# tyfeld/MMaDA-Parallel

Measured on NVIDIA B200. Metric: denoised_tokens_per_sec, higher is better.
Workload: dtype bf16

## Files before the change

### mmada_parallel_b200/csrc/gemm.cu

```cuda
#include "gemm_epilogue.cuh"

#include <stdlib.h>

#include <map>
#include <mutex>
#include <utility>

namespace mmdp {

static constexpr int BM = 128, BK = 64;
static constexpr int kABytes = BM * BK * 2;
static constexpr int kGemmThreads = 256;
template <int BN> struct GemmCfg {
    static constexpr int kBBytes = BN * BK * 2;
    static constexpr int kStageBytes = kABytes + kBBytes;
    static constexpr int kStages = (BN == 256) ? 4 : 5;
    static constexpr int kScatBytes = 4 * kScatStageFloats * 4;
    static constexpr int kSmem = kStages * kStageBytes + 1024  + 256  + kScatBytes;
};

template <int EPI, int BN>
__global__ void __launch_bounds__(kGemmThreads, 1)
gemm_bf16_kernel(const __grid_constant__ CUtensorMap tmA, const __grid_constant__ CUtensorMap tmB, const GemmParams p) {
    constexpr int kStages = GemmCfg<BN>::kStages;
// ... 192 lines not shown
void set_gemm_splitk_mode(int m) { set_opt("gemm_splitk", m); }

static GemmPlan plan_gemm(int epi, int M, int N, int K) {
    const int mode = gemm_splitk_mode();
    const int g = num_sms();
    const int num_k = (K + BK - 1) / BK;
    const bool flexible = epi == EPI_PLAIN || epi == EPI_RESID || epi == EPI_F32;
    const bool may_split = num_k >= 4 && (mode >= 2 || (mode == 1 && epi == EPI_RESID));
    GemmPlan best{256, 0, 0, 0, 0};
    double best_cost = 1e30;
    for (int bn : {256, 192}) {
        if (bn == 192 && !flexible) continue;
        const int tiles = ((M + BM - 1) / BM) * ((N + bn - 1) / bn);
        GemmPlan pl{bn, tiles < g ? tiles : g, 0, 0, 0};
        double waves;
        const int full = tiles >= g ? (tiles / g) * g : 0;
        const int tail = tiles - full;
        waves = (double)((tiles + g - 1) / g);
        if (may_split && tail > 0 && tail * 2 <= g) {
            int splits = g / tail;
            if (splits > num_k / 2) splits = num_k / 2;
            if (splits > kSkMaxSplits) splits = kSkMaxSplits;
            if (splits >= 2) {
                const int kb_per = (num_k + splits - 1) / splits;
                splits = (num_k + kb_per - 1) / kb_per;
                const double exch = mode >= 3 ? 0.0 : 12.0 / num_k + 0.04;
                const double split_waves = (double)(full / g) + (double)kb_per / num_k + exch;
                if (split_waves < waves) {
                    pl.tail = tail; pl.splits = splits; pl.kb_per = kb_per;
                    pl.grid = full > 0 ? g : tail * splits;
                    waves = split_waves;
                }
            }
        }
        const double cost = waves * bn * (bn == 192 ? 1.04 : 1.0);
        if (cost < best_cost) { best_cost = cost; best = pl; }
    }
    return best;
}

struct SkWorkspace { float* ws; int* cnt; };
static std::map<std::pair<int, cudaStream_t>, SkWorkspace> g_sk;
static std::mutex g_sk_mu;
static int splitk_workspace(cudaStream_t stream, SkWorkspace* out) {
    int dev = 0;
    MMDP_CUDA(cudaGetDevice(&dev));
    std::lock_guard<std::mutex> lk(g_sk_mu);
    auto key = std::make_pair(dev, stream);
    auto it = g_sk.find(key);
    if (it != g_sk.end()) { *out = it->second; return 0; }
    const size_t units = 256;
    SkWorkspace w{nullptr, nullptr};
    MMDP_CUDA(cudaMalloc(&w.ws, units * BM * 256 * sizeof(float)));
    MMDP_CUDA(cudaMalloc(&w.cnt, 2 * units * sizeof(int)));
    MMDP_CUDA(cudaMemsetAsync(w.cnt, 0, 2 * units * sizeof(int), stream));
    g_sk.emplace(key, w);
    *out = w;
    return 0;
}

int gemm_pair_mode() { return opt(OPT_GEMM_PAIR); }
void set_gemm_pair_mode(int on) { set_opt("gemm_pair", (on == 2) ? 2 : (on ? 1 : 0)); }

int gemm_bf16(int epi, const __nv_bfloat16* A, int lda, const __nv_bfloat16* W, int ldw, int M, int N, int K,
              __nv_bfloat16* C, int ldc, const __nv_bfloat16* resid, int ldr, const QkvRopeArgs* qa,
              cudaStream_t stream, const GemmScatter* sc) {
    if (sc && epi != EPI_F32) return set_error("gemm: the scatter epilogue belongs to MMDP_EPI_F32");
    if (sc && (sc->rows_per_rank <= 0 || sc->slot < 0 || sc->slot > 7 || (M + sc->rows_per_rank - 1) / sc->rows_per_rank > 8))
        return set_error("gemm: bad scatter layout");
    if (M <= 0 || N <= 0 || K <= 0) return set_error("gemm: empty problem");
    if ((lda % 8) || (ldw % 8) || (K % 8)) return set_error("gemm: lda/ldw/K must be multiples of 8 (16-byte TMA strides)");
    if ((reinterpret_cast<uintptr_t>(A) & 15) || (reinterpret_cast<uintptr_t>(W) & 15))
        return set_error("gemm: A/W must be 16-byte aligned");
    switch (epi) {
        case EPI_PLAIN:
            if (!C || (ldc % 8) || (N % 8)) return set_error("gemm: C null or ldc/N not multiple of 8");
            break;
        case EPI_RESID:
            if (!C || !resid || (ldc % 8) || (ldr % 8) || (N % 8)) return set_error("gemm: bad residual epilogue args");
            break;
        case EPI_F32:
            if ((!C && !sc) || (ldc % 4) || (N % 4)) return set_error("gemm: fp32 output needs ldc/N multiples of 4");
            break;
        case EPI_SWIGLU:
            if (!C || (ldc % 8) || (N % 256)) return set_error("gemm: swiglu needs N % 256 == 0 (interleaved gate/up tiles)");
            break;
        case EPI_QKVROPE:
            if (!qa) return set_error("gemm: qkv epilogue needs QkvRopeArgs");
            if (qa->d_model % 256 || N != 3 * qa->d_model || qa->d_model != qa->n_heads * 128)
                return set_error("gemm: qkv epilogue needs head_dim 128, d_model % 256 == 0, N == 3*d_model");
            if (qa->pos_map ? (qa->Tq <= 0 || M % qa->Tq) : (!qa->chunked && (M % qa->L))) return set_error("gemm: qkv epilogue needs M == B*L (or B*Tq with a position map)");
            break;
        default:
            return set_error("gemm: unknown epilogue");
    }
    const int pm = gemm_pair_mode();
    if ((pm == 1 && M > 256) || (pm == 2 && M >= 4096 && N >= 8192)) return gemm_bf16_pair(epi, A, lda, W, ldw, M, N, K, C, ldc, resid, ldr, qa, stream, sc);
    GemmParams p{};
    p.M = M; p.N = N; p.K = K;
    p.C = C; p.ldc = ldc; p.resid = resid; p.ldr = ldr;
    GemmPlan pl = plan_gemm(epi, M, N, K);
    if (qa && qa->pos_map && pl.tail > 0) {
        pl.tail = 0; pl.splits = 0; pl.kb_per = 0;
        const int t = ((M + BM - 1) / BM) * ((N + pl.bn - 1) / pl.bn);
        pl.grid = t < num_sms() ? t : num_sms();
    }
    if (sc) {
        if (pl.tail > 0) { pl.tail = 0; pl.splits = 0; pl.kb_per = 0; const int t = ((M + BM - 1) / BM) * ((N + pl.bn - 1) / pl.bn); pl.grid = t < num_sms() ? t : num_sms(); }
        for (int r = 0; r < 8; ++r) p.scat_dst[r] = sc->dst[r];
        p.scat_R = sc->rows_per_rank; p.scat_slot = sc->slot;
// ... 45 lines not shown
```

### mmada_parallel_b200/csrc/gemm2.cu

```cuda
#include "gemm_epilogue.cuh"

namespace mmdp {

static constexpr int P_BM = 128, P_BK = 64;
static constexpr int kPABytes = P_BM * P_BK * 2;
static constexpr int kPairThreads = 256;
template <int BN> struct PairCfg {
    static constexpr int kBHalfBytes = (BN / 2) * P_BK * 2;
    static constexpr int kStageBytes = kPABytes + kBHalfBytes;
    static constexpr int kStages = (BN == 256) ? 6 : 7;
    static constexpr int kSmem = kStages * kStageBytes + 1024 + 256 + 4 * kScatStageFloats * 4;
    template <int EPI> static constexpr bool can_split() { return BN == 256 && (EPI == EPI_PLAIN || EPI == EPI_RESID || EPI == EPI_QKVROPE); }
};

__device__ __forceinline__ uint32_t cluster_ctarank() {
    uint32_t r;
    asm volatile("mov.u32 %0, %%cluster_ctarank;" : "=r"(r));
    return r;
}
__device__ __forceinline__ void cluster_sync_all() {
    asm volatile("barrier.cluster.arrive.release.aligned;\n\tbarrier.cluster.wait.acquire.aligned;" ::: "memory");
}
__device__ __forceinline__ uint32_t mapa_u32(uint32_t smem_addr, uint32_t rank) {
    uint32_t r;
    asm volatile("mapa.shared::cluster.u32 %0, %1, %2;" : "=r"(r) : "r"(smem_addr), "r"(rank));
    return r;
}
__device__ __forceinline__ void mbar_arrive_cluster(uint32_t cluster_addr) {
    asm volatile("mbarrier.arrive.shared::cluster.b64 _, [%0];" ::"r"(cluster_addr) : "memory");
}
template <uint32_t kCols>
__device__ __forceinline__ void tmem_alloc_pair(uint32_t* smem_dst) {
    asm volatile("tcgen05.alloc.cta_group::2.sync.aligned.shared::cta.b32 [%0], %1;" ::"r"(smem_u32(smem_dst)), "n"(kCols) : "memory");
    asm volatile("tcgen05.relinquish_alloc_permit.cta_group::2.sync.aligned;" ::: "memory");
}
template <uint32_t kCols>
__device__ __forceinline__ void tmem_dealloc_pair(uint32_t taddr) {
    asm volatile("tcgen05.dealloc.cta_group::2.sync.aligned.b32 %0, %1;" ::"r"(taddr), "n"(kCols) : "memory");
}
__device__ __forceinline__ void tma_load_2d_pair(void* smem_dst, const CUtensorMap* tm, uint32_t leader_bar_cluster_addr, int c0, int c1) {
    asm volatile(
        "cp.async.bulk.tensor.2d.cta_group::2.shared::cluster.global.mbarrier::complete_tx::bytes [%0], [%1, {%3, %4}], [%2];"
        ::"r"(smem_u32(smem_dst)), "l"(reinterpret_cast<uint64_t>(tm)), "r"(leader_bar_cluster_addr), "r"(c0), "r"(c1)
        : "memory");
}
__device__ __forceinline__ void umma_bf16_ss_pair(uint32_t d_tmem, uint64_t a_desc, uint64_t b_desc, uint32_t idesc, uint32_t acc) {
    asm volatile(
        "{\n\t.reg .pred p;\n\t"
        "setp.ne.b32 p, %4, 0;\n\t"
        "tcgen05.mma.cta_group::2.kind::f16 [%0], %1, %2, %3, p;\n\t}"
        ::"r"(d_tmem), "l"(a_desc), "l"(b_desc), "r"(idesc), "r"(acc)
        : "memory");
}
__device__ __forceinline__ void umma_commit_pair(uint64_t* bar) {
    const uint16_t mask = 3;
    asm volatile("tcgen05.commit.cta_group::2.mbarrier::arrive::one.shared::cluster.multicast::cluster.b64 [%0], %1;"
                 ::"r"(smem_u32(bar)), "h"(mask)
                 : "memory");
}

template <int EPI, int BN>
__global__ void __cluster_dims__(2, 1, 1) __launch_bounds__(kPairThreads, 1)
gemm_pair_kernel(const __grid_constant__ CUtensorMap tmA, const __grid_constant__ CUtensorMap tmB,
                 const __grid_constant__ CUtensorMap tmBh, const __grid_constant__ CUtensorMap tmAh, const GemmParams p) {
    constexpr int kStages = PairCfg<BN>::kStages;
    constexpr int kStageBytes = PairCfg<BN>::kStageBytes;
    static_assert(EPI == EPI_PLAIN || EPI == EPI_RESID || EPI == EPI_F32 || BN == 256, "fused QKV / SwiGLU epilogues need 256-wide tiles");
    extern __shared__ uint8_t smem_raw[];
    uint8_t* smem = reinterpret_cast<uint8_t*>((reinterpret_cast<uintptr_t>(smem_raw) + 1023) & ~uintptr_t(1023));
    uint64_t* full_bar = reinterpret_cast<uint64_t*>(smem + kStages * kStageBytes);
    uint64_t* empty_bar = full_bar + kStages;
    uint64_t* tmem_full = empty_bar + kStages;
    uint64_t* tmem_empty = tmem_full + 2;
    uint32_t* tmem_ptr = reinterpret_cast<uint32_t*>(tmem_empty + 2);
    float* scat_stage = reinterpret_cast<float*>(smem + kStages * kStageBytes + 256);

    const int warp = threadIdx.x >> 5;
    const int lane = threadIdx.x & 31;
    const uint32_t rank = cluster_ctarank();
    const bool leader = rank == 0;

    if (warp == 0 && lane == 0) {
        tma_prefetch_desc(&tmA);
        tma_prefetch_desc(&tmB);
    }
    if (warp == 1 && lane == 0) {
        for (int s = 0; s < kStages; ++s) {
            mbar_init(&full_bar[s], 2);
            mbar_init(&empty_bar[s], 1);
        }
        for (int s = 0; s < 2; ++s) {
            mbar_init(&tmem_full[s], 1);
            mbar_init(&tmem_empty[s], 8);
        }
        fence_barrier_init();
    }
    cluster_sync_all();
    if (warp == 2) tmem_alloc_pair<512>(tmem_ptr);
    tcgen05_fence_before();
    cluster_sync_all();
    tcgen05_fence_after();
    const uint32_t tmem_base = *tmem_ptr;
    pdl_launch_dependents();
    pdl_wait();

    const int num_m = (p.M + 2 * P_BM - 1) / (2 * P_BM);
    const int num_n = (p.N + BN - 1) / BN;
    const int num_k = (p.K + P_BK - 1) / P_BK;
    const int num_tiles = num_m * num_n;
    const int cluster_id = blockIdx.x >> 1, num_clusters = gridDim.x >> 1;
    constexpr bool kCanSplit = PairCfg<BN>::template can_split<EPI>();
    const int t_full = kCanSplit ? num_tiles - p.nsplit_tail : num_tiles;
    const int num_units = t_full + 2 * (num_tiles - t_full);
    constexpr bool kMTail = EPI == EPI_SWIGLU && BN == 256;
    auto decode = [&](int unit, int& m_blk, int& n_blk, bool& mhalf) {
        n_blk = unit / num_m;
        const int o = unit - n_blk * num_m;
        mhalf = false;
        m_blk = o;
        if (kMTail && p.mtail) {
            const int sp = (n_blk / p.mt_period) % num_m;
            mhalf = o == sp;
            m_blk = mhalf ? num_m - 1 : (o < sp ? o : o - 1);
        }
    };

    if (warp == 0) {
        if (elect_one_sync()) {
            int s = 0;
            uint32_t ph = 0;
            for (int unit = cluster_id; unit < num_units; unit += num_clusters) {
                const bool half = kCanSplit && unit >= t_full;
                const int tile = half ? t_full + ((unit - t_full) >> 1) : unit;
                int m_blk, n_blk;
                bool mhalf;
                decode(tile, m_blk, n_blk, mhalf);
                const int row0 = mhalf ? m_blk * 2 * P_BM + (int)rank * (P_BM / 2) : m_blk * 2 * P_BM + (int)rank * P_BM;
                const int wrow0 = half ? n_blk * BN + ((unit - t_full) & 1) * (BN / 2) + (int)rank * (BN / 4) : n_blk * BN + (int)rank * (BN / 2);
                const uint32_t tx = half ? 2 * (kPABytes + PairCfg<BN>::kBHalfBytes / 2)
                                         : (mhalf ? 2 * (kPABytes / 2 + PairCfg<BN>::kBHalfBytes) : 2 * kStageBytes);
                for (int kb = 0; kb < num_k; ++kb) {
                    mbar_wait(&empty_bar[s], ph ^ 1);
                    const uint32_t leader_full = mapa_u32(smem_u32(&full_bar[s]), 0);
                    if (leader) {
                        mbar_expect_tx(&full_bar[s], tx);
                    } else {
                        mbar_arrive_cluster(leader_full);
                    }
                    uint8_t* sa = smem + s * kStageBytes;
                    if (kMTail && mhalf) {
                        tma_load_2d_pair(sa, &tmAh, leader_full, kb * P_BK, row0);
                        tma_load_2d_pair(sa + kPABytes, &tmBh, leader_full, kb * P_BK, n_blk * BN + (int)rank * (BN / 4));
                        tma_load_2d_pair(sa + kPABytes + PairCfg<BN>::kBHalfBytes / 2, &tmBh, leader_full, kb * P_BK, n_blk * BN + BN / 2 + (int)rank * (BN / 4));
                    } else {
                        tma_load_2d_pair(sa, &tmA, leader_full, kb * P_BK, row0);
                        tma_load_2d_pair(sa + kPABytes, half ? &tmBh : &tmB, leader_full, kb * P_BK, wrow0);
                    }
                    if (++s == kStages) { s = 0; ph ^= 1; }
                }
            }
        }
        __syncwarp();
    } else if (warp == 1) {
        if (leader && elect_one_sync()) {
            constexpr uint32_t idesc_whole = umma_idesc_bf16(2 * P_BM, BN);
            constexpr uint32_t idesc_half = umma_idesc_bf16(2 * P_BM, kCanSplit ? BN / 2 : BN);
            int s = 0;
            uint32_t ph = 0;
            int as = 0;
            uint32_t aph = 0;
            constexpr uint32_t idesc_mhalf = umma_idesc_bf16(P_BM, BN);
            for (int unit = cluster_id; unit < num_units; unit += num_clusters) {
                uint32_t idesc = (kCanSplit && unit >= t_full) ? idesc_half : idesc_whole;
                if (kMTail && p.mtail) {
                    int m_blk, n_blk;
                    bool mhalf;
                    decode(unit, m_blk, n_blk, mhalf);
                    if (mhalf) idesc = idesc_mhalf;
                }
                mbar_wait(&tmem_empty[as], aph ^ 1);
                tcgen05_fence_after();
                const uint32_t d_tmem = tmem_base + as * BN;
                for (int kb = 0; kb < num_k; ++kb) {
                    mbar_wait(&full_bar[s], ph);
                    tcgen05_fence_after();
                    const uint32_t sa = smem_u32(smem + s * kStageBytes);
                    const uint64_t adesc = umma_desc_kmajor_sw128(sa);
                    const uint64_t bdesc = umma_desc_kmajor_sw128(sa + kPABytes);
#pragma unroll
                    for (int k = 0; k < P_BK / 16; ++k)
                        umma_bf16_ss_pair(d_tmem, adesc + (k * 2), bdesc + (k * 2), idesc, (kb | k) != 0);
                    umma_commit_pair(&empty_bar[s]);
                    if (kb == num_k - 1) umma_commit_pair(&tmem_full[as]);
                    if (++s == kStages) { s = 0; ph ^= 1; }
                }
                if (++as == 2) { as = 0; aph ^= 1; }
            }
        }
        __syncwarp();
    } else if (warp >= 4) {
        const int ew = warp - 4;
        int as = 0;
        uint32_t aph = 0;
        for (int unit = cluster_id; unit < num_units; unit += num_clusters) {
            const bool half = kCanSplit && unit >= t_full;
            const int tile = half ? t_full + ((unit - t_full) >> 1) : unit;
            int m_blk, n_blk;
            bool mhalf;
            decode(tile, m_blk, n_blk, mhalf);
            mbar_wait(&tmem_full[as], aph);
            tcgen05_fence_after();
            const uint32_t tbase = tmem_base + (static_cast<uint32_t>(ew * 32) << 16) + as * BN;
            if (kMTail && mhalf) {
                const int ln = ew * 32 + lane, hq = ln >> 6;
                const int row = m_blk * 2 * P_BM + (int)rank * (P_BM / 2) + (ln & 63);
                const bool row_ok = row < p.M;
#pragma unroll 1
                for (int c = 0; c < 2; ++c) {
                    uint32_t g[32], u[32];
                    tmem_ld_32x32b_x32(tbase + c * 32, g);
                    tmem_ld_32x32b_x32(tbase + 64 + c * 32, u);
                    tmem_ld_wait();
                    swiglu_store32(p, g, u, row, row_ok, n_blk * 128 + hq * 64 + c * 32);
                }
            } else {
            const int row = m_blk * 2 * P_BM + (int)rank * P_BM + ew * 32 + lane;
            const bool row_ok = row < p.M;
            if constexpr (kCanSplit) {
                if (half)
                    gemm_epilogue_tile<EPI, BN / 2>(p, tbase, row, row_ok, 2 * n_blk + ((unit - t_full) & 1), scat_stage + ew * kScatStageFloats);
                else
                    gemm_epilogue_tile<EPI, BN>(p, tbase, row, row_ok, n_blk, scat_stage + ew * kScatStageFloats);
            } else {
                gemm_epilogue_tile<EPI, BN>(p, tbase, row, row_ok, n_blk, scat_stage + ew * kScatStageFloats);
            }
            }
            tcgen05_fence_before();
            __syncwarp();
            if (lane == 0) mbar_arrive_cluster(mapa_u32(smem_u32(&tmem_empty[as]), 0));
            if (++as == 2) { as = 0; aph ^= 1; }
        }
        if constexpr (EPI == EPI_F32) {
            if (p.scat_R > 0) __threadfence_system();
        }
    }

    tcgen05_fence_before();
    cluster_sync_all();
    if (warp == 2) {
        tcgen05_fence_after();
        tmem_dealloc_pair<512>(tmem_base);
    }
}

template <int EPI, int BN>
static int launch_pair(const CUtensorMap& tmA, const CUtensorMap& tmB, const CUtensorMap& tmBh, const CUtensorMap& tmAh, GemmParams& p, cudaStream_t stream) {
    static unsigned long long attr_set = 0;
    int dev = 0;
    MMDP_CUDA(cudaGetDevice(&dev));
    if (!(attr_set >> (dev & 63) & 1ull)) {
        MMDP_CUDA(cudaFuncSetAttribute(gemm_pair_kernel<EPI, BN>, cudaFuncAttributeMaxDynamicSharedMemorySize, PairCfg<BN>::kSmem));
        attr_set |= 1ull << (dev & 63);
    }
    const int num_tiles = ((p.M + 2 * P_BM - 1) / (2 * P_BM)) * ((p.N + BN - 1) / BN);
    const int pairs = num_sms() / 2;
    const int grid = 2 * (num_tiles < pairs ? num_tiles : pairs);
    const int tail = num_tiles % pairs;
    p.nsplit_tail = (PairCfg<BN>::template can_split<EPI>() && opt(OPT_GEMM_NSPLIT_TAIL) && num_tiles > pairs && tail > 0 &&
                     2 * tail <= pairs && p.N % BN == 0) ? tail : 0;
    const int num_m = (p.M + 2 * P_BM - 1) / (2 * P_BM), m_rem = p.M - (num_m - 1) * 2 * P_BM;
    p.mtail = (EPI == EPI_SWIGLU && BN == 256 && opt(OPT_GEMM_MTAIL) && num_m >= 2 && m_rem <= P_BM && p.N % BN == 0 && num_tiles > pairs) ? 1 : 0;
    if (p.mtail) {
        int a = num_m, b = pairs;
        while (b) { const int t = a % b; a = b; b = t; }
        p.mt_period = pairs / a;
    }
    LaunchScope ls(LK_GEMM, 2.0 * p.M * (double)p.N * p.K, stream);
    MMDP_CUDA(launch_ex(gemm_pair_kernel<EPI, BN>, dim3(grid), dim3(kPairThreads), PairCfg<BN>::kSmem, stream, pdl_mode() != 0, false, tmA, tmB,
                        (p.nsplit_tail || p.mtail) ? tmBh : tmB, p.mtail ? tmAh : tmA, p));
    return 0;
}

static int pick_pair_tile_n(int M, int N) {
    const int g = num_sms() / 2;
    const long long m_tiles = (M + 2 * P_BM - 1) / (2 * P_BM);
    const long long w256 = (m_tiles * ((N + 255) / 256) + g - 1) / g * 256 * 100;
    const long long w192 = (m_tiles * ((N + 191) / 192) + g - 1) / g * 192 * 102;
    return w192 < w256 ? 192 : 256;
}

int gemm_bf16_pair(int epi, const __nv_bfloat16* A, int lda, const __nv_bfloat16* W, int ldw, int M, int N, int K,
                   __nv_bfloat16* C, int ldc, const __nv_bfloat16* resid, int ldr, const QkvRopeArgs* qa, cudaStream_t stream,
                   const GemmScatter* sc) {
    GemmParams p{};
    p.M = M; p.N = N; p.K = K;
    p.C = C; p.ldc = ldc; p.resid = resid; p.ldr = ldr;
    if (sc) {
        for (int r = 0; r < 8; ++r) p.scat_dst[r] = sc->dst[r];
        p.scat_R = sc->rows_per_rank; p.scat_slot = sc->slot;
    }
    const int bn = (epi == EPI_PLAIN || epi == EPI_RESID || epi == EPI_F32) ? pick_pair_tile_n(M, N) : 256;
    CUtensorMap tmA, tmB;
    if (make_tmap_2d_bf16(&tmA, A, (uint64_t)M, (uint64_t)K, (uint64_t)lda, P_BM, P_BK)) return -1;
    if (make_tmap_2d_bf16(&tmB, W, (uint64_t)N, (uint64_t)K, (uint64_t)ldw, bn / 2, P_BK)) return -1;
    CUtensorMap tmBh = tmB;
    if (bn == 256 && epi != EPI_F32 && make_tmap_2d_bf16(&tmBh, W, (uint64_t)N, (uint64_t)K, (uint64_t)ldw, bn / 4, P_BK)) return -1;
    CUtensorMap tmAh = tmA;
    if (epi == EPI_SWIGLU && make_tmap_2d_bf16(&tmAh, A, (uint64_t)M, (uint64_t)K, (uint64_t)lda, P_BM / 2, P_BK)) return -1;
    switch (epi) {
        case EPI_PLAIN:
            return bn == 192 ? launch_pair<EPI_PLAIN, 192>(tmA, tmB, tmBh, tmAh, p, stream) : launch_pair<EPI_PLAIN, 256>(tmA, tmB, tmBh, tmAh, p, stream);
        case EPI_RESID:
            return bn == 192 ? launch_pair<EPI_RESID, 192>(tmA, tmB, tmBh, tmAh, p, stream) : launch_pair<EPI_RESID, 256>(tmA, tmB, tmBh, tmAh, p, stream);
        case EPI_F32:
            return bn == 192 ? launch_pair<EPI_F32, 192>(tmA, tmB, tmBh, tmAh, p, stream) : launch_pair<EPI_F32, 256>(tmA, tmB, tmBh, tmAh, p, stream);
        case EPI_SWIGLU:
            return launch_pair<EPI_SWIGLU, 256>(tmA, tmB, tmBh, tmAh, p, stream);
        case EPI_QKVROPE:
            p.q = qa->q; p.k = qa->k; p.vt = qa->vt; p.cos_tab = qa->cos_tab; p.sin_tab = qa->sin_tab;
            p.L = qa->L; p.Lpad = qa->Lpad; p.d_model = qa->d_model; p.n_heads = qa->n_heads;
            p.pos_map = qa->pos_map; p.Tq = qa->Tq; p.row0 = qa->row0;
            return launch_pair<EPI_QKVROPE, 256>(tmA, tmB, tmBh, tmAh, p, stream);
        default:
            return set_error("gemm_pair: unknown epilogue");
    }
}

}
```

### mmada_parallel_b200/csrc/gemm_epilogue.cuh

```cuda
#pragma once
#include "mmdp_internal.h"
#include "ptx.cuh"

namespace mmdp {

struct GemmParams {
    int M, N, K;
    __nv_bfloat16* C;
    int ldc;
    const __nv_bfloat16* resid;
    int ldr;
    __nv_bfloat16* q;
    __nv_bfloat16* k;
    __nv_bfloat16* vt;
    const float* cos_tab;
    const float* sin_tab;
    int L, Lpad, d_model, n_heads;
    const int* pos_map;
    int Tq;
    int row0;
    int sk_tail, sk_splits, sk_kb_per;
    float* sk_ws;
    int* sk_cnt;
    int l2pf, l2pf_mod;
    float* scat_dst[8];
    int scat_R, scat_slot;
    int group_m;
    int nsplit_tail;
    int mtail, mt_period;
};

__host__ __device__ __forceinline__ void gemm_tile_coords(int tl, int num_m, int num_n, int group_m, int& m_blk, int& n_blk) {
    if (group_m <= 0 || group_m >= num_m) {
        m_blk = tl % num_m;
        n_blk = tl / num_m;
    } else {
        const int per_group = group_m * num_n;
        const int gid = tl / per_group, r = tl - gid * per_group;
        const int first = gid * group_m;
        const int gsz = (num_m - first < group_m) ? num_m - first : group_m;
        m_blk = first + r % gsz;
        n_blk = r / gsz;
    }
}

__device__ __forceinline__ void store_bf16x32(__nv_bfloat16* dst, const uint32_t (&p)[16], int ncols_valid) {
    uint4* d4 = reinterpret_cast<uint4*>(dst);
#pragma unroll
    for (int i = 0; i < 4; ++i) {
        if (i * 8 < ncols_valid) d4[i] = make_uint4(p[4 * i], p[4 * i + 1], p[4 * i + 2], p[4 * i + 3]);
    }
}

__device__ __forceinline__ void swiglu_store32(const GemmParams& p, const uint32_t (&g)[32], const uint32_t (&u)[32], int row, bool row_ok, int col0) {
    const int nvalid = p.N / 2 - col0;
    if (row_ok && nvalid > 0) {
        uint32_t pk[16];
#pragma unroll
        for (int i = 0; i < 16; ++i) {
            float o[2];
#pragma unroll
            for (int h = 0; h < 2; ++h) {
                float gg = bf16_round(__uint_as_float(g[2 * i + h]));
                float uu = bf16_round(__uint_as_float(u[2 * i + h]));
                float s = bf16_round(__fdiv_rn(gg, __fadd_rn(1.0f, expf(-gg))));
                o[h] = __fmul_rn(s, uu);
            }
            pk[i] = pack_bf16x2(o[0], o[1]);
        }
        store_bf16x32(p.C + (size_t)row * p.ldc + col0, pk, nvalid);
    }
}

static constexpr int kScatStageFloats = 32 * 36;

template <int EPI, int BN>
__device__ __forceinline__ void gemm_epilogue_tile(const GemmParams& p, uint32_t tbase, int row, bool row_ok, int n_blk,
                                                   float* stage = nullptr) {
            const int n0 = n_blk * BN;
            if constexpr (EPI == EPI_F32) {
              if (p.scat_R > 0) {
                const int lane = threadIdx.x & 31;
// ... 139 lines not shown
                    }
                }
            }
}

static constexpr int kSkMaxSplits = 8;

template <int BN, int NV>
__device__ __forceinline__ void sk_sum(const float4* __restrict__ tile_ws, int S, int row, const int (&col4)[NV], float4 (&acc)[NV]) {
    constexpr int kSplitStride = (BN / 4) * 128;
    constexpr int kBatch = 4;
    static_assert(kSkMaxSplits % kBatch == 0, "batches");
#pragma unroll
    for (int b0 = 0; b0 < kSkMaxSplits; b0 += kBatch) {
        if (b0 < S) {
            float4 part[kBatch][NV];
#pragma unroll
            for (int j = 0; j < kBatch; ++j)
                if (b0 + j < S) {
#pragma unroll
                    for (int v = 0; v < NV; ++v) part[j][v] = __ldcg(tile_ws + (size_t)(b0 + j) * kSplitStride + col4[v] * 128 + row);
                }
#pragma unroll
            for (int j = 0; j < kBatch; ++j)
                if (b0 + j < S) {
#pragma unroll
                    for (int v = 0; v < NV; ++v) {
                        if (b0 + j == 0) {
                            acc[v] = part[0][v];
                        } else {
                            acc[v].x = __fadd_rn(acc[v].x, part[j][v].x);
                            acc[v].y = __fadd_rn(acc[v].y, part[j][v].y);
                            acc[v].z = __fadd_rn(acc[v].z, part[j][v].z);
                            acc[v].w = __fadd_rn(acc[v].w, part[j][v].w);
                        }
                    }
                }
        }
    }
}

template <int BN>
__device__ __forceinline__ void sk_publish(float4* __restrict__ slot_ws, uint32_t tbase, int rit) {
#pragma unroll 1
    for (int c = 0; c < BN / 32; ++c) {
        uint32_t v[32];
        tmem_ld_32x32b_x32(tbase + c * 32, v);
        tmem_ld_wait();
#pragma unroll
        for (int i = 0; i < 8; ++i)
            slot_ws[(size_t)(c * 8 + i) * 128 + rit] = make_float4(__uint_as_float(v[4 * i]), __uint_as_float(v[4 * i + 1]),
                                                                  __uint_as_float(v[4 * i + 2]), __uint_as_float(v[4 * i + 3]));
    }
}

template <int EPI, int BN>
__device__ __forceinline__ void sk_finish(const GemmParams& p, const float4* __restrict__ tile_ws, int S, int unit_s, int m_blk,
                                          int n_blk, int tid) {
    const int r0 = (128 * unit_s) / S, r1 = (128 * (unit_s + 1)) / S;
    const int nrows = r1 - r0;
    const int n0 = n_blk * BN;
    if constexpr (EPI == EPI_PLAIN || EPI == EPI_RESID || EPI == EPI_F32) {
        constexpr int G = BN / 8;
        for (int idx = tid; idx < nrows * G; idx += 128) {
            const int g = idx / nrows, rit = r0 + idx - g * nrows;
            const int row = m_blk * 128 + rit, col = n0 + 8 * g;
            if (row >= p.M || col >= p.N) continue;
            const int col4[2] = {2 * g, 2 * g + 1};
            float4 a[2];
            sk_sum<BN, 2>(tile_ws, S, rit, col4, a);
            if constexpr (EPI == EPI_F32) {
                float4* d = reinterpret_cast<float4*>(reinterpret_cast<float*>(p.C) + (size_t)row * p.ldc + col);
                d[0] = a[0];
                if (col + 4 < p.N) d[1] = a[1];
            } else {
                const float f[8] = {a[0].x, a[0].y, a[0].z, a[0].w, a[1].x, a[1].y, a[1].z, a[1].w};
                uint32_t o[4];
                if constexpr (EPI == EPI_RESID) {
                    const uint4 rv = *reinterpret_cast<const uint4*>(p.resid + (size_t)row * p.ldr + col);
                    const uint32_t rr[4] = {rv.x, rv.y, rv.z, rv.w};
#pragma unroll
                    for (int i = 0; i < 4; ++i)
                        o[i] = pack_bf16x2(__fadd_rn(bf16_lo(rr[i]), bf16_round(f[2 * i])), __fadd_rn(bf16_hi(rr[i]), bf16_round(f[2 * i + 1])));
                } else {
#pragma unroll
                    for (int i = 0; i < 4; ++i) o[i] = pack_bf16x2(f[2 * i], f[2 * i + 1]);
                }
                *reinterpret_cast<uint4*>(p.C + (size_t)row * p.ldc + col) = make_uint4(o[0], o[1], o[2], o[3]);
            }
        }
    } else if constexpr (EPI == EPI_SWIGLU) {
        constexpr int G = 16;
        for (int idx = tid; idx < nrows * G; idx += 128) {
            const int g = idx / nrows, rit = r0 + idx - g * nrows;
            const int row = m_blk * 128 + rit, col = n_blk * 128 + 8 * g;
            if (row >= p.M || col >= p.N / 2) continue;
            const int col4[4] = {2 * g, 2 * g + 1, 32 + 2 * g, 32 + 2 * g + 1};
            float4 a[4];
            sk_sum<BN, 4>(tile_ws, S, rit, col4, a);
            const float gt[8] = {a[0].x, a[0].y, a[0].z, a[0].w, a[1].x, a[1].y, a[1].z, a[1].w};
            const float up[8] = {a[2].x, a[2].y, a[2].z, a[2].w, a[3].x, a[3].y, a[3].z, a[3].w};
            float o[8];
#pragma unroll
            for (int i = 0; i < 8; ++i) {
                const float gg = bf16_round(gt[i]), uu = bf16_round(up[i]);
                const float sl = bf16_round(__fdiv_rn(gg, __fadd_rn(1.0f, expf(-gg))));
// ... 62 lines not shown
```

### mmada_parallel_b200/csrc/mmdp_internal.h

```cpp
#pragma once
#include <cuda.h>
#include <cuda_bf16.h>
#include <cuda_runtime.h>
#include <stdint.h>
#include <stdio.h>

namespace mmdp {

enum Epilogue { EPI_PLAIN = 0, EPI_RESID = 1, EPI_QKVROPE = 2, EPI_SWIGLU = 3, EPI_F32 = 4 };

int set_error(const char* fmt, ...);
const char* last_error();
int num_sms();

enum LaunchKind { LK_GEMM = 0, LK_ATTN = 1, LK_ROW = 2, LK_SAMPLE = 3, LK_COUNT = 4 };
struct LaunchScope {
    LaunchScope(int kind, double work, cudaStream_t s);
    ~LaunchScope();
    int idx;
    cudaStream_t stream;
};
void prof_enable(int on);
int prof_summary(double* ms, double* work, long long* launches);
long long launch_count(int reset);
// ... 35 lines not shown
    do {                                                                                             \
        cudaError_t _e = (expr);                                                                     \
        if (_e != cudaSuccess)                                                                       \
            return ::mmdp::set_error("%s:%d: %s -> %s", __FILE__, __LINE__, #expr, cudaGetErrorString(_e)); \
    } while (0)

int make_tmap_2d_bf16(CUtensorMap* out, const void* base, uint64_t rows, uint64_t cols, uint64_t ld, uint32_t box_rows,
                      uint32_t box_cols);
int make_tmap_2d(CUtensorMap* out, const void* base, int elem_bytes, uint64_t rows, uint64_t cols, uint64_t ld,
                 uint32_t box_rows, uint32_t box_cols);

int conv_tf32(const float* A, int lda, long long a_rows, const float* W, int M, int N, int K, int T, const int* shifts,
              float* C, int ldc, const float* R, int ldr, const float* bias, int bias_along_m, float alpha, int pad_w,
              int pad_h, int scatter_w, int scatter_h, cudaStream_t stream);
int gn_swish(const float* x, float* y, int B, int C, int H, int W, double* stats_ws, const float* gamma, const float* beta,
             float eps, int swish, int compact, cudaStream_t stream);
int upsample2x(const float* x, float* y, int B, int C, int H, int W, cudaStream_t stream);
int softmax_rows_ld(float* s, int rows, int n, int ld, cudaStream_t stream);
int zero_border(float* y, int B, int C, int H, int W, cudaStream_t stream);
int lfq_to_padded(const int64_t* ids, float* z, int B, int H, int W, int bits, int Cpad, cudaStream_t stream);
int nchw_to_padded(const float* x, float* y, int B, int C, int Cpad, int H, int W, cudaStream_t stream);
int downsample_pick(const float* src, float* dst, int B, int C, int H, int W, cudaStream_t stream);
int lfq_indices(const float* z, int64_t* ids, int B, int h, int w, int bits, int ld, cudaStream_t stream);
int padded_to_nchw(const float* x, float* y, int B, int C, int ld, int H, int W, cudaStream_t stream);

struct QkvRopeArgs {
    __nv_bfloat16* q;
    __nv_bfloat16* k;
    __nv_bfloat16* vt;
    const float* cos_tab;
    const float* sin_tab;
    int L, Lpad, d_model, n_heads;
    const int* pos_map = nullptr;
    int Tq = 0;
    int chunked = 0;
    int row0 = 0;
};

struct GemmScatter {
    float* dst[8];
    int rows_per_rank, slot;
};

int gemm_bf16(int epi, const __nv_bfloat16* A, int lda, const __nv_bfloat16* W, int ldw, int M, int N, int K,
              __nv_bfloat16* C, int ldc, const __nv_bfloat16* resid, int ldr, const QkvRopeArgs* qa,
              cudaStream_t stream, const GemmScatter* sc = nullptr);

int gemm_bf16_pair(int epi, const __nv_bfloat16* A, int lda, const __nv_bfloat16* W, int ldw, int M, int N, int K,
                   __nv_bfloat16* C, int ldc, const __nv_bfloat16* resid, int ldr, const QkvRopeArgs* qa, cudaStream_t stream,
                   const GemmScatter* sc = nullptr);
int gemm_pair_mode();
void set_gemm_pair_mode(int on);
int gemm_splitk_mode();
void set_gemm_splitk_mode(int mode);

int attention_fwd(const __nv_bfloat16* q, const __nv_bfloat16* k, const __nv_bfloat16* vt, __nv_bfloat16* out, int B,
                  int H, int L, int Lpad, float scale, cudaStream_t stream, int Lq = 0);

int embed_rows(const int64_t* ids, const __nv_bfloat16* wte, __nv_bfloat16* x, int M, int d, int64_t vocab,
               cudaStream_t stream, int* err = nullptr);
int rmsnorm(const __nv_bfloat16* x, int ldx, const __nv_bfloat16* w, __nv_bfloat16* y, int ldy, int M, int d, float eps,
            cudaStream_t stream);
int resid_add_f32(__nv_bfloat16* x, int ldx, const float* partial, int ldp, int M, int d, cudaStream_t stream);
int rmsnorm_rows(const __nv_bfloat16* x, int ldx, const int* rows, const __nv_bfloat16* w, __nv_bfloat16* y, int ldy,
                 int M, int d, float eps, cudaStream_t stream, int src_rows = 0x7fffffff, int* err = nullptr, int row_lo = 0, int row_hi = 0, int row_mod = 0);

int text_step(const __nv_bfloat16* cond, const __nv_bfloat16* uncond, int64_t ld, int R, int V, float text_cfg,
              const __nv_bfloat16* unoise, int64_t ld_noise, float temperature, int64_t* ids_text, int64_t mask_id,
              int k, int64_t* x0_ws, double* conf_ws, cudaStream_t stream, const double* unoise64 = nullptr);
int image_step(int variant, const __nv_bfloat16* cond, const __nv_bfloat16* unc_a, const __nv_bfloat16* unc_b, int64_t ld,
               int N, int C, float s_a, float s_b, const __nv_bfloat16* qnoise, const __nv_bfloat16* conf_noise,
               float temp, int sched_len, int64_t* ids, const int* pos, int64_t mask_id, int64_t vq_offset,
               int32_t* sampled_ws, float* selp_ws, uint8_t* unknown_ws, __nv_bfloat16* probs_out,
               int32_t* mask_len_out, uint8_t* masking_out, cudaStream_t stream);
int image_remask(int variant, int N, const int32_t* sampled, const float* selp, const uint8_t* unknown,
                 const __nv_bfloat16* conf_noise, float temp, int sched_len, int64_t* ids, const int* pos, int64_t mask_id,
                 int64_t vq_offset, int32_t* mask_len_out, uint8_t* masking_out, cudaStream_t stream, int k_direct = -1);
int image_step_t2i(const __nv_bfloat16* cond, const __nv_bfloat16* uncond, int64_t ld, int N, int C, float cfg,
                   const __nv_bfloat16* gumbel_u, float tau, const __nv_bfloat16* conf_u, float temperature, int keep_n,
                   int64_t* ids, const int* pos, int64_t mask_id, int64_t vq_offset, int32_t* sampled_ws, float* selp_ws,
                   uint8_t* unknown_ws, uint8_t* masking_out, cudaStream_t stream);
int lfq_decode(const int64_t* ids, float* zq, int B, int N, int bits, cudaStream_t stream);
int tp_reduce_norm(const float* recv_local, int rows_per_rank, int n_src, uint16_t* const* xn, uint32_t* const* flags, int n_ranks,
                   int my_rank, uint16_t* x_shard, const uint16_t* w, int row0, int nrows, int d, float eps, uint32_t epoch,
                   unsigned int* done_counter, cudaStream_t stream);

}
```

Baseline: 214.8.

## Add stream-K style K-split hand-off scheduling to paired-CTA GEMM

Replaces round-robin tile assignment in the 2-CTA cluster GEMM with a planner that can divide the last partial wave's K work evenly across clusters. A cluster finishing the head of a split tile publishes its fp32 accumulator to global memory and raises a flag. The cluster doing the tail spins on that flag and reloads the partial sum into tensor memory before continuing the MMA. This aims to remove wave-quantization idle time, at the cost of global-memory hand-off traffic and cross-cluster spin waits that rely on all clusters being co-resident, which an occupancy check guards.

```diff
diff --git a/mmada_parallel_b200/csrc/gemm.cu b/mmada_parallel_b200/csrc/gemm.cu
--- a/mmada_parallel_b200/csrc/gemm.cu
+++ b/mmada_parallel_b200/csrc/gemm.cu
@@ -268,10 +268,19 @@
     const size_t units = 256;
     SkWorkspace w{nullptr, nullptr};
     MMDP_CUDA(cudaMalloc(&w.ws, units * BM * 256 * sizeof(float)));
-    MMDP_CUDA(cudaMalloc(&w.cnt, 2 * units * sizeof(int)));
-    MMDP_CUDA(cudaMemsetAsync(w.cnt, 0, 2 * units * sizeof(int), stream));
+    MMDP_CUDA(cudaMalloc(&w.cnt, 3 * units * sizeof(int)));
+    MMDP_CUDA(cudaMemsetAsync(w.cnt, 0, 3 * units * sizeof(int), stream));
     g_sk.emplace(key, w);
     *out = w;
+    return 0;
+}
+
+int pair_handoff_workspace(cudaStream_t stream, int slots, float** ws, int** flags) {
+    if (slots > 256) return set_error("gemm_pair: %d hand-off slots exceed the workspace", slots);
+    SkWorkspace w;
+    if (splitk_workspace(stream, &w)) return -1;
+    *ws = w.ws;
+    *flags = w.cnt + 2 * 256;
     return 0;
 }
 
diff --git a/mmada_parallel_b200/csrc/gemm2.cu b/mmada_parallel_b200/csrc/gemm2.cu
--- a/mmada_parallel_b200/csrc/gemm2.cu
+++ b/mmada_parallel_b200/csrc/gemm2.cu
@@ -72,7 +72,8 @@
     uint64_t* empty_bar = full_bar + kStages;
     uint64_t* tmem_full = empty_bar + kStages;
     uint64_t* tmem_empty = tmem_full + 2;
-    uint32_t* tmem_ptr = reinterpret_cast<uint32_t*>(tmem_empty + 2);
+    uint64_t* tail_ready = tmem_empty + 2;
+    uint32_t* tmem_ptr = reinterpret_cast<uint32_t*>(tail_ready + 1);
     float* scat_stage = reinterpret_cast<float*>(smem + kStages * kStageBytes + 256);
 
     const int warp = threadIdx.x >> 5;
@@ -93,6 +94,7 @@
             mbar_init(&tmem_full[s], 1);
             mbar_init(&tmem_empty[s], 8);
         }
+        mbar_init(tail_ready, 8);
         fence_barrier_init();
     }
     cluster_sync_all();
@@ -108,10 +110,11 @@
     const int num_n = (p.N + BN - 1) / BN;
     const int num_k = (p.K + P_BK - 1) / P_BK;
     const int num_tiles = num_m * num_n;
-    const int cluster_id = blockIdx.x >> 1, num_clusters = gridDim.x >> 1;
+    const int cluster_id = blockIdx.x >> 1;
     constexpr bool kCanSplit = PairCfg<BN>::template can_split<EPI>();
     const int t_full = kCanSplit ? num_tiles - p.nsplit_tail : num_tiles;
     const int num_units = t_full + 2 * (num_tiles - t_full);
+    const int num_items = pair_num_items(p.ps, cluster_id, num_units);
     constexpr bool kMTail = EPI == EPI_SWIGLU && BN == 256;
     auto decode = [&](int unit, int& m_blk, int& n_blk, bool& mhalf) {
         n_blk = unit / num_m;
@@ -129,7 +132,9 @@
         if (elect_one_sync()) {
             int s = 0;
             uint32_t ph = 0;
-            for (int unit = cluster_id; unit < num_units; unit += num_clusters) {
+            for (int i = 0; i < num_items; ++i) {
+                const PairItem it = pair_item(p.ps, cluster_id, i);
+                const int unit = it.unit;
                 const bool half = kCanSplit && unit >= t_full;
                 const int tile = half ? t_full + ((unit - t_full) >> 1) : unit;
                 int m_blk, n_blk;
@@ -139,7 +144,7 @@
                 const int wrow0 = half ? n_blk * BN + ((unit - t_full) & 1) * (BN / 2) + (int)rank * (BN / 4) : n_blk * BN + (int)rank * (BN / 2);
                 const uint32_t tx = half ? 2 * (kPABytes + PairCfg<BN>::kBHalfBytes / 2)
                                          : (mhalf ? 2 * (kPABytes / 2 + PairCfg<BN>::kBHalfBytes) : 2 * kStageBytes);
-                for (int kb = 0; kb < num_k; ++kb) {
+                for (int kb = it.kb0; kb < it.kb1; ++kb) {
                     mbar_wait(&empty_bar[s], ph ^ 1);
                     const uint32_t leader_full = mapa_u32(smem_u32(&full_bar[s]), 0);
                     if (leader) {
@@ -170,7 +175,9 @@
             int as = 0;
             uint32_t aph = 0;
             constexpr uint32_t idesc_mhalf = umma_idesc_bf16(P_BM, BN);
-            for (int unit = cluster_id; unit < num_units; unit += num_clusters) {
+            for (int i = 0; i < num_items; ++i) {
+                const PairItem it = pair_item(p.ps, cluster_id, i);
+                const int unit = it.unit;
                 uint32_t idesc = (kCanSplit && unit >= t_full) ? idesc_half : idesc_whole;
                 if (kMTail && p.mtail) {
                     int m_blk, n_blk;
@@ -179,9 +186,10 @@
                     if (mhalf) idesc = idesc_mhalf;
                 }
                 mbar_wait(&tmem_empty[as], aph ^ 1);
+                if (it.kind == PAIR_TAIL) mbar_wait(tail_ready, 0);
                 tcgen05_fence_after();
                 const uint32_t d_tmem = tmem_base + as * BN;
-                for (int kb = 0; kb < num_k; ++kb) {
+                for (int kb = it.kb0; kb < it.kb1; ++kb) {
                     mbar_wait(&full_bar[s], ph);
                     tcgen05_fence_after();
                     const uint32_t sa = smem_u32(smem + s * kStageBytes);
@@ -191,7 +199,7 @@
                     for (int k = 0; k < P_BK / 16; ++k)
                         umma_bf16_ss_pair(d_tmem, adesc + (k * 2), bdesc + (k * 2), idesc, (kb | k) != 0);
                     umma_commit_pair(&empty_bar[s]);
-                    if (kb == num_k - 1) umma_commit_pair(&tmem_full[as]);
+                    if (kb == it.kb1 - 1) umma_commit_pair(&tmem_full[as]);
                     if (++s == kStages) { s = 0; ph ^= 1; }
                 }
                 if (++as == 2) { as = 0; aph ^= 1; }
@@ -202,16 +210,53 @@
         const int ew = warp - 4;
         int as = 0;
         uint32_t aph = 0;
-        for (int unit = cluster_id; unit < num_units; unit += num_clusters) {
+        const int rit = ew * 32 + lane;
+        for (int i = 0; i < num_items; ++i) {
+            const PairItem it = pair_item(p.ps, cluster_id, i);
+            const int unit = it.unit;
             const bool half = kCanSplit && unit >= t_full;
             const int tile = half ? t_full + ((unit - t_full) >> 1) : unit;
             int m_blk, n_blk;
             bool mhalf;
             decode(tile, m_blk, n_blk, mhalf);
+            const bool next_tail = i + 1 < num_items && pair_item(p.ps, cluster_id, i + 1).kind == PAIR_TAIL;
+            auto load_tail = [&]() {
+                const int src = 2 * (cluster_id - 1) + (int)rank;
+                if (rit == 0) {
+                    int* flag = p.ho_flag + src;
+                    uint32_t spins = 0;
+                    int v;
+                    while (true) {
+                        asm volatile("ld.acquire.gpu.global.b32 %0, [%1];" : "=r"(v) : "l"(flag) : "memory");
+                        if (v != 0) break;
+                        if (++spins > (1u << 24)) {
+                            printf("mmdp: gemm_pair K hand-off timeout (cluster %d)\n", cluster_id);
+                            break;
+                        }
+                        __nanosleep(64);
+                    }
+                    *flag = 0;
+                    __threadfence();
+                }
+                asm volatile("bar.sync 1, 128;" ::: "memory");
+                const uint32_t tnext = tmem_base + (static_cast<uint32_t>(ew * 32) << 16) + (as ^ 1) * BN;
+                sk_restore<BN>(reinterpret_cast<const float4*>(p.ho_ws) + (size_t)src * (BN / 4) * 128, tnext, rit);
+                tcgen05_fence_before();
+                __syncwarp();
+                if (lane == 0) mbar_arrive_cluster(mapa_u32(smem_u32(tail_ready), 0));
+            };
+            if (next_tail && it.kind != PAIR_HEAD) load_tail();
             mbar_wait(&tmem_full[as], aph);
             tcgen05_fence_after();
             const uint32_t tbase = tmem_base + (static_cast<uint32_t>(ew * 32) << 16) + as * BN;
-            if (kMTail && mhalf) {
+            if (it.kind == PAIR_HEAD) {
+                const int dst = 2 * cluster_id + (int)rank;
+                sk_publish<BN>(reinterpret_cast<float4*>(p.ho_ws) + (size_t)dst * (BN / 4) * 128, tbase, rit);
+                __threadfence();
+                asm volatile("bar.sync 1, 128;" ::: "memory");
+                if (rit == 0) asm volatile("st.release.gpu.global.b32 [%0], %1;" ::"l"(p.ho_flag + dst), "r"(1) : "memory");
+                if (next_tail) load_tail();
+            } else if (kMTail && mhalf) {
                 const int ln = ew * 32 + lane, hq = ln >> 6;
                 const int row = m_blk * 2 * P_BM + (int)rank * (P_BM / 2) + (ln & 63);
                 const bool row_ok = row < p.M;
@@ -254,39 +299,40 @@
 }
 
 template <int EPI, int BN>
-static int launch_pair(const CUtensorMap& tmA, const CUtensorMap& tmB, const CUtensorMap& tmBh, const CUtensorMap& tmAh, GemmParams& p, cudaStream_t stream) {
+static int launch_pair(const CUtensorMap& tmA, const CUtensorMap& tmB, const CUtensorMap& tmBh, const CUtensorMap& tmAh, GemmParams& p,
+                       const PairPlan& pl, cudaStream_t stream) {
     static unsigned long long attr_set = 0;
+    static int max_clusters[64] = {};
     int dev = 0;
     MMDP_CUDA(cudaGetDevice(&dev));
     if (!(attr_set >> (dev & 63) & 1ull)) {
         MMDP_CUDA(cudaFuncSetAttribute(gemm_pair_kernel<EPI, BN>, cudaFuncAttributeMaxDynamicSharedMemorySize, PairCfg<BN>::kSmem));
+        cudaLaunchConfig_t cfg{};
+        cudaLaunchAttribute at{};
+        at.id = cudaLaunchAttributeClusterDimension;
+        at.val.clusterDim.x = 2; at.val.clusterDim.y = 1; at.val.clusterDim.z = 1;
+        cfg.gridDim = dim3(num_sms()); cfg.blockDim = dim3(kPairThreads); cfg.dynamicSmemBytes = PairCfg<BN>::kSmem;
+        cfg.attrs = &at; cfg.numAttrs = 1;
+        int n = 0;
+        if (cudaOccupancyMaxActiveClusters(&n, gemm_pair_kernel<EPI, BN>, &cfg) != cudaSuccess) { (void)cudaGetLastError(); n = 0; }
+        max_clusters[dev & 63] = n;
         attr_set |= 1ull << (dev & 63);
     }
     const int num_tiles = ((p.M + 2 * P_BM - 1) / (2 * P_BM)) * ((p.N + BN - 1) / BN);
-    const int pairs = num_sms() / 2;
+    PairPlan use = pl;
+    if (use.sched.sk_units > 0 && max_clusters[dev & 63] < use.sched.C)
+        use = pair_plan_round_robin(EPI, p.M, p.N, p.K, use.sched.C, BN, opt(OPT_GEMM_NSPLIT_TAIL) != 0, opt(OPT_GEMM_MTAIL) != 0);
+    if (use.sched.sk_units > 0 && pair_handoff_workspace(stream, 2 * use.sched.C, &p.ho_ws, &p.ho_flag)) return -1;
+    p.ps = use.sched;
+    p.nsplit_tail = use.nsplit_tail;
+    p.mtail = use.mtail;
+    p.mt_period = use.mt_period;
+    const int pairs = use.sched.C;
     const int grid = 2 * (num_tiles < pairs ? num_tiles : pairs);
-    const int tail = num_tiles % pairs;
-    p.nsplit_tail = (PairCfg<BN>::template can_split<EPI>() && opt(OPT_GEMM_NSPLIT_TAIL) && num_tiles > pairs && tail > 0 &&
-                     2 * tail <= pairs && p.N % BN == 0) ? tail : 0;
-    const int num_m = (p.M + 2 * P_BM - 1) / (2 * P_BM), m_rem = p.M - (num_m - 1) * 2 * P_BM;
-    p.mtail = (EPI == EPI_SWIGLU && BN == 256 && opt(OPT_GEMM_MTAIL) && num_m >= 2 && m_rem <= P_BM && p.N % BN == 0 && num_tiles > pairs) ? 1 : 0;
-    if (p.mtail) {
-        int a = num_m, b = pairs;
-        while (b) { const int t = a % b; a = b; b = t; }
-        p.mt_period = pairs / a;
-    }
     LaunchScope ls(LK_GEMM, 2.0 * p.M * (double)p.N * p.K, stream);
     MMDP_CUDA(launch_ex(gemm_pair_kernel<EPI, BN>, dim3(grid), dim3(kPairThreads), PairCfg<BN>::kSmem, stream, pdl_mode() != 0, false, tmA, tmB,
                         (p.nsplit_tail || p.mtail) ? tmBh : tmB, p.mtail ? tmAh : tmA, p));
     return 0;
-}
-
-static int pick_pair_tile_n(int M, int N) {
-    const int g = num_sms() / 2;
-    const long long m_tiles = (M + 2 * P_BM - 1) / (2 * P_BM);
-    const long long w256 = (m_tiles * ((N + 255) / 256) + g - 1) / g * 256 * 100;
-    const long long w192 = (m_tiles * ((N + 191) / 192) + g - 1) / g * 192 * 102;
-    return w192 < w256 ? 192 : 256;
 }
 
 int gemm_bf16_pair(int epi, const __nv_bfloat16* A, int lda, const __nv_bfloat16* W, int ldw, int M, int N, int K,
@@ -299,7 +345,9 @@
         for (int r = 0; r < 8; ++r) p.scat_dst[r] = sc->dst[r];
         p.scat_R = sc->rows_per_rank; p.scat_slot = sc->slot;
     }
-    const int bn = (epi == EPI_PLAIN || epi == EPI_RESID || epi == EPI_F32) ? pick_pair_tile_n(M, N) : 256;
+    const PairPlan pl = pair_plan(epi, M, N, K, num_sms() / 2, gemm_splitk_mode() != 0, opt(OPT_GEMM_NSPLIT_TAIL) != 0,
+                                  opt(OPT_GEMM_MTAIL) != 0);
+    const int bn = pl.bn;
     CUtensorMap tmA, tmB;
     if (make_tmap_2d_bf16(&tmA, A, (uint64_t)M, (uint64_t)K, (uint64_t)lda, P_BM, P_BK)) return -1;
     if (make_tmap_2d_bf16(&tmB, W, (uint64_t)N, (uint64_t)K, (uint64_t)ldw, bn / 2, P_BK)) return -1;
@@ -309,18 +357,18 @@
     if (epi == EPI_SWIGLU && make_tmap_2d_bf16(&tmAh, A, (uint64_t)M, (uint64_t)K, (uint64_t)lda, P_BM / 2, P_BK)) return -1;
     switch (epi) {
         case EPI_PLAIN:
-            return bn == 192 ? launch_pair<EPI_PLAIN, 192>(tmA, tmB, tmBh, tmAh, p, stream) : launch_pair<EPI_PLAIN, 256>(tmA, tmB, tmBh, tmAh, p, stream);
+            return bn == 192 ? launch_pair<EPI_PLAIN, 192>(tmA, tmB, tmBh, tmAh, p, pl, stream) : launch_pair<EPI_PLAIN, 256>(tmA, tmB, tmBh, tmAh, p, pl, stream);
         case EPI_RESID:
-            return bn == 192 ? launch_pair<EPI_RESID, 192>(tmA, tmB, tmBh, tmAh, p, stream) : launch_pair<EPI_RESID, 256>(tmA, tmB, tmBh, tmAh, p, stream);
+            return bn == 192 ? launch_pair<EPI_RESID, 192>(tmA, tmB, tmBh, tmAh, p, pl, stream) : launch_pair<EPI_RESID, 256>(tmA, tmB, tmBh, tmAh, p, pl, stream);
         case EPI_F32:
-            return bn == 192 ? launch_pair<EPI_F32, 192>(tmA, tmB, tmBh, tmAh, p, stream) : launch_pair<EPI_F32, 256>(tmA, tmB, tmBh, tmAh, p, stream);
+            return bn == 192 ? launch_pair<EPI_F32, 192>(tmA, tmB, tmBh, tmAh, p, pl, stream) : launch_pair<EPI_F32, 256>(tmA, tmB, tmBh, tmAh, p, pl, stream);
         case EPI_SWIGLU:
-            return launch_pair<EPI_SWIGLU, 256>(tmA, tmB, tmBh, tmAh, p, stream);
+            return launch_pair<EPI_SWIGLU, 256>(tmA, tmB, tmBh, tmAh, p, pl, stream);
         case EPI_QKVROPE:
             p.q = qa->q; p.k = qa->k; p.vt = qa->vt; p.cos_tab = qa->cos_tab; p.sin_tab = qa->sin_tab;
             p.L = qa->L; p.Lpad = qa->Lpad; p.d_model = qa->d_model; p.n_heads = qa->n_heads;
             p.pos_map = qa->pos_map; p.Tq = qa->Tq; p.row0 = qa->row0;
-            return launch_pair<EPI_QKVROPE, 256>(tmA, tmB, tmBh, tmAh, p, stream);
+            return launch_pair<EPI_QKVROPE, 256>(tmA, tmB, tmBh, tmAh, p, pl, stream);
         default:
             return set_error("gemm_pair: unknown epilogue");
     }
diff --git a/mmada_parallel_b200/csrc/gemm_epilogue.cuh b/mmada_parallel_b200/csrc/gemm_epilogue.cuh
--- a/mmada_parallel_b200/csrc/gemm_epilogue.cuh
+++ b/mmada_parallel_b200/csrc/gemm_epilogue.cuh
@@ -1,4 +1,5 @@
 #pragma once
+#include "gemm_schedule.cuh"
 #include "mmdp_internal.h"
 #include "ptx.cuh"
 
@@ -28,6 +29,9 @@
     int group_m;
     int nsplit_tail;
     int mtail, mt_period;
+    PairSched ps;
+    float* ho_ws;
+    int* ho_flag;
 };
 
 __host__ __device__ __forceinline__ void gemm_tile_coords(int tl, int num_m, int num_n, int group_m, int& m_blk, int& n_blk) {
@@ -273,6 +277,22 @@
             slot_ws[(size_t)(c * 8 + i) * 128 + rit] = make_float4(__uint_as_float(v[4 * i]), __uint_as_float(v[4 * i + 1]),
                                                                   __uint_as_float(v[4 * i + 2]), __uint_as_float(v[4 * i + 3]));
     }
+}
+
+template <int BN>
+__device__ __forceinline__ void sk_restore(const float4* __restrict__ slot_ws, uint32_t tbase, int rit) {
+#pragma unroll 1
+    for (int c = 0; c < BN / 32; ++c) {
+        uint32_t v[32];
+#pragma unroll
+        for (int i = 0; i < 8; ++i) {
+            const float4 f = __ldcg(slot_ws + (size_t)(c * 8 + i) * 128 + rit);
+            v[4 * i] = __float_as_uint(f.x); v[4 * i + 1] = __float_as_uint(f.y);
+            v[4 * i + 2] = __float_as_uint(f.z); v[4 * i + 3] = __float_as_uint(f.w);
+        }
+        tmem_st_32x32b_x32(tbase + c * 32, v);
+    }
+    tmem_st_wait();
 }
 
 template <int EPI, int BN>
diff --git a/mmada_parallel_b200/csrc/gemm_schedule.cuh b/mmada_parallel_b200/csrc/gemm_schedule.cuh
--- /dev/null
+++ b/mmada_parallel_b200/csrc/gemm_schedule.cuh
@@ -0,0 +1,113 @@
+#pragma once
+#include "mmdp_internal.h"
+
+namespace mmdp {
+
+struct PairSched {
+    int C;
+    int num_k;
+    int dp_waves;
+    int sk_units;
+};
+
+enum PairItemKind { PAIR_WHOLE = 0, PAIR_HEAD = 1, PAIR_TAIL = 2 };
+struct PairItem { int unit, kb0, kb1, kind; };
+
+__host__ __device__ __forceinline__ void pair_sk_range(const PairSched& s, int c, long long& lo, long long& hi) {
+    const long long W = (long long)s.sk_units * s.num_k;
+    lo = W * c / s.C;
+    hi = W * (c + 1) / s.C;
+}
+
+__host__ __device__ __forceinline__ int pair_num_items(const PairSched& s, int c, int num_units) {
+    if (s.sk_units == 0) return c < num_units ? (num_units - c + s.C - 1) / s.C : 0;
+    long long lo, hi;
+    pair_sk_range(s, c, lo, hi);
+    const int has_head = hi % s.num_k != 0, has_tail = lo % s.num_k != 0;
+    const int first_whole = (int)((lo + s.num_k - 1) / s.num_k), end_whole = (int)(hi / s.num_k);
+    return has_head + s.dp_waves + (end_whole - first_whole) + has_tail;
+}
+
+__host__ __device__ __forceinline__ PairItem pair_item(const PairSched& s, int c, int i) {
+    if (s.sk_units == 0) return PairItem{c + i * s.C, 0, s.num_k, PAIR_WHOLE};
+    long long lo, hi;
+    pair_sk_range(s, c, lo, hi);
+    const int sk0 = s.dp_waves * s.C;
+    if (hi % s.num_k != 0) {
+        if (i == 0) return PairItem{sk0 + (int)(hi / s.num_k), 0, (int)(hi % s.num_k), PAIR_HEAD};
+        --i;
+    }
+    if (i < s.dp_waves) return PairItem{c + i * s.C, 0, s.num_k, PAIR_WHOLE};
+    i -= s.dp_waves;
+    const int first_whole = (int)((lo + s.num_k - 1) / s.num_k), end_whole = (int)(hi / s.num_k);
+    if (i < end_whole - first_whole) return PairItem{sk0 + first_whole + i, 0, s.num_k, PAIR_WHOLE};
+    return PairItem{sk0 + (int)(lo / s.num_k), (int)(lo % s.num_k), s.num_k, PAIR_TAIL};
+}
+
+static constexpr double kPairSkHandoff = 0.05;
+
+struct PairPlan {
+    int bn;
+    int nsplit_tail;
+    int mtail, mt_period;
+    PairSched sched;
+};
+
+inline int pair_num_m(int M) { return (M + 255) / 256; }
+
+inline PairPlan pair_plan_round_robin(int epi, int M, int N, int K, int C, int bn, bool nsplit, bool mtail) {
+    PairPlan pl{};
+    pl.bn = bn;
+    const int num_m = pair_num_m(M), num_tiles = num_m * ((N + bn - 1) / bn);
+    pl.sched = PairSched{C, (K + 63) / 64, 0, 0};
+    const bool can_split = bn == 256 && (epi == EPI_PLAIN || epi == EPI_RESID || epi == EPI_QKVROPE);
+    const int tail = num_tiles % C;
+    pl.nsplit_tail = (can_split && nsplit && num_tiles > C && tail > 0 && 2 * tail <= C && N % bn == 0) ? tail : 0;
+    const int m_rem = M - (num_m - 1) * 256;
+    pl.mtail = (epi == EPI_SWIGLU && bn == 256 && mtail && num_m >= 2 && m_rem <= 128 && N % bn == 0 && num_tiles > C) ? 1 : 0;
+    if (pl.mtail) {
+        int a = num_m, b = C;
+        while (b) { const int t = a % b; a = b; b = t; }
+        pl.mt_period = C / a;
+    }
+    return pl;
+}
+
+inline int pair_pick_tile_n_round_robin(int M, int N, int C) {
+    const long long m_tiles = pair_num_m(M);
+    const long long w256 = (m_tiles * ((N + 255) / 256) + C - 1) / C * 256 * 100;
+    const long long w192 = (m_tiles * ((N + 191) / 192) + C - 1) / C * 192 * 102;
+    return w192 < w256 ? 192 : 256;
+}
+
+inline PairPlan pair_plan(int epi, int M, int N, int K, int C, bool balanced, bool nsplit, bool mtail) {
+    const bool flexible = epi == EPI_PLAIN || epi == EPI_RESID || epi == EPI_F32;
+    if (!balanced || epi == EPI_F32) {
+        const int bn = flexible ? pair_pick_tile_n_round_robin(M, N, C) : 256;
+        return pair_plan_round_robin(epi, M, N, K, C, bn, nsplit, mtail);
+    }
+    PairPlan best{};
+    double best_cost = 1e30;
+    for (int bn : {256, 192}) {
+        if (bn == 192 && !flexible) continue;
+        const double w = bn == 256 ? 1.0 : 0.75 * 1.02;
+        const int U = pair_num_m(M) * ((N + bn - 1) / bn);
+        PairPlan rr = pair_plan_round_robin(epi, M, N, K, C, bn, nsplit, mtail);
+        double waves = (double)((U + C - 1) / C);
+        if (rr.nsplit_tail) waves = U / C + 0.5;
+        if (waves * w < best_cost) { best_cost = waves * w; best = rr; }
+        if (U > C && U % C != 0) {
+            const double sk_waves = (double)U / C + kPairSkHandoff;
+            if (sk_waves * w < best_cost) {
+                best_cost = sk_waves * w;
+                best = PairPlan{};
+                best.bn = bn;
+                const int dp = U / C - 1;
+                best.sched = PairSched{C, (K + 63) / 64, dp, U - dp * C};
+            }
+        }
+    }
+    return best;
+}
+
+}
diff --git a/mmada_parallel_b200/csrc/mmdp_internal.h b/mmada_parallel_b200/csrc/mmdp_internal.h
--- a/mmada_parallel_b200/csrc/mmdp_internal.h
+++ b/mmada_parallel_b200/csrc/mmdp_internal.h
@@ -111,6 +111,7 @@
 int gemm_pair_mode();
 void set_gemm_pair_mode(int on);
 int gemm_splitk_mode();
+int pair_handoff_workspace(cudaStream_t stream, int slots, float** ws, int** flags);
 void set_gemm_splitk_mode(int mode);
 
 int attention_fwd(const __nv_bfloat16* q, const __nv_bfloat16* k, const __nv_bfloat16* vt, __nv_bfloat16* out, int B,
```

After: 209.0 (median of 6 runs). 2.7% lower.
